# Nicolo2277/Vivim

Measured on AMD Instinct MI355X. Metric: frames/sec fwd+bwd, 256x256 clip=5 3-class, higher is better.
Workload: dtype bf16

## Files before the change

### include/vivim_hip.h

```cpp
#ifndef VIVIM_HIP_H
#define VIVIM_HIP_H

#include <stddef.h>
#include <stdint.h>

#ifdef __cplusplus
extern "C" {
#endif

#define VIVIM_ABI_VERSION 8

typedef enum { VIVIM_F32 = 0, VIVIM_F16 = 1, VIVIM_BF16 = 2 } vivim_dtype_t;

enum {
    VIVIM_OK = 0,
    VIVIM_ERR_INVALID = 1,
    VIVIM_ERR_UNSUPPORTED = 2,
    VIVIM_ERR_LAUNCH = 3
};

typedef struct {
    int32_t batch, dim, seqlen, dstate, n_groups;
    int32_t itype;
    int32_t is_variable_B;
// ... 119 lines not shown
    const void *weight;
    const void *bias;
    void *out;
} vivim_conv_update_params;

typedef struct {
    int32_t batch, dim, dstate;
    int32_t itype;
    int32_t stype;
    int32_t dt_softplus;
    int64_t state_batch_stride, state_d_stride, state_n_stride;
    int64_t x_batch_stride, x_d_stride, dt_batch_stride, dt_d_stride;
    int64_t A_d_stride, A_n_stride;
    int64_t B_batch_stride, B_n_stride, C_batch_stride, C_n_stride;
    int64_t z_batch_stride, z_d_stride, out_batch_stride, out_d_stride;
    void *state;
    const void *x, *dt;
    const void *A;
    const void *B, *C;
    const void *D;
    const void *z;
    const void *dt_bias;
    void *out;
} vivim_state_update_params;

typedef struct {
    int32_t batch, seqlen, channels;
    int32_t itype, otype;
    float eps;
    int64_t x_batch_stride, x_c_stride;
    int64_t y_batch_stride, y_token_stride;
    int64_t dx_batch_stride, dx_c_stride;
    const void *x;
    const void *weight, *bias;
    void *y;
    void *mean, *rstd;
    const void *dy;
    void *dx;
    void *dweight, *dbias;
    void *workspace;
} vivim_layernorm_params;

typedef struct {
    int32_t groups, m, n, k;
    int32_t itype;
    int32_t _pad0;
    int64_t a_group_stride, a_row_stride;
    int64_t b_group_stride, b_row_stride;
    int64_t out_group_stride, out_row_stride;
    const void *a, *b;
    void *out;
} vivim_wgrad_nt_params;

int vivim_abi_version(void);
const char *vivim_last_error(void);

size_t vivim_sizeof(int which);

int vivim_scan_ckpt_len(const vivim_ssm_fwd_params *f);
int vivim_scan_chunk_len(int itype);

size_t vivim_scan_bwd_workspace_bytes(const vivim_ssm_fwd_params *f);
size_t vivim_scan_fwd_workspace_bytes(const vivim_ssm_fwd_params *f);

int vivim_set_tuning(int which, int value);

int vivim_selective_scan_fwd(const vivim_ssm_fwd_params *p, void *stream);
int vivim_selective_scan_bwd(const vivim_ssm_bwd_params *p, void *stream);
int vivim_causal_conv1d_fwd(const vivim_conv_fwd_params *p, void *stream);
int vivim_causal_conv1d_bwd(const vivim_conv_bwd_params *p, void *stream);
int vivim_dwconv_fwd(const vivim_dwconv_params *p, void *stream);
int vivim_dwconv_wgrad(const vivim_dwconv_wgrad_params *p, void *stream);
int vivim_dir_scatter(const vivim_dir_params *p, void *stream);
int vivim_dir_gather(const vivim_dir_params *p, void *stream);
int vivim_causal_conv1d_update(const vivim_conv_update_params *p, void *stream);
int vivim_selective_state_update(const vivim_state_update_params *p, void *stream);
int vivim_layernorm_cm_fwd(const vivim_layernorm_params *p, void *stream);
int vivim_layernorm_cm_bwd(const vivim_layernorm_params *p, void *stream);
size_t vivim_layernorm_bwd_workspace_bytes(const vivim_layernorm_params *p);
int vivim_wgrad_nt(const vivim_wgrad_nt_params *p, void *stream);

size_t vivim_scan_bwd_det_workspace_bytes(const vivim_ssm_fwd_params *f);
size_t vivim_scan_bwd_det_call_workspace_bytes(const vivim_ssm_bwd_params *p);
int vivim_selective_scan_bwd_det(const vivim_ssm_bwd_params *p, void *det_ws, size_t det_ws_bytes, void *stream);

size_t vivim_causal_conv1d_bwd_det_workspace_bytes(const vivim_conv_fwd_params *f);
int vivim_causal_conv1d_bwd_det(const vivim_conv_bwd_params *p, void *det_ws, size_t det_ws_bytes, void *stream);
size_t vivim_dwconv_wgrad_det_workspace_bytes(const vivim_dwconv_wgrad_params *p);
int vivim_dwconv_wgrad_det(const vivim_dwconv_wgrad_params *p, void *det_ws, size_t det_ws_bytes, void *stream);

#ifdef __cplusplus
}
#endif
#endif
```

### vivim_amd/_lib.py

```python
import ctypes
import os
import subprocess

_HERE = os.path.dirname(os.path.abspath(__file__))
CSRC = os.path.join(_HERE, "csrc")
SO_PATH = os.environ.get("VIVIM_LIB") or os.path.join(CSRC, "libvivim_hip.so")

i32, i64, vp = ctypes.c_int32, ctypes.c_int64, ctypes.c_void_p

F32, F16, BF16 = 0, 1, 2


class SsmFwdParams(ctypes.Structure):
    _fields_ = (
        [(n, i32) for n in ("batch", "dim", "seqlen", "dstate", "n_groups", "itype", "is_variable_B",
                            "is_variable_C", "delta_softplus", "_pad0")]
        + [(n, i64) for n in ("u_batch_stride", "u_d_stride", "delta_batch_stride", "delta_d_stride",
                              "z_batch_stride", "z_d_stride", "out_batch_stride", "out_d_stride",
                              "out_z_batch_stride", "out_z_d_stride", "A_d_stride", "A_dstate_stride",
                              "B_batch_stride", "B_group_stride", "B_dstate_stride",
                              "C_batch_stride", "C_group_stride", "C_dstate_stride")]
        + [(n, vp) for n in ("u", "delta", "A", "B", "C", "D", "delta_bias", "z", "out", "out_z", "x", "workspace")]
        + [("workspace_bytes", i64)]
    )
# ... 38 lines not shown
        + [(n, i64) for n in ("x_batch_stride", "x_token_stride", "y_batch_stride", "y_token_stride")]
        + [(n, vp) for n in ("x", "wt", "bias", "y")]
        + [("act", i32), ("_pad1", i32), ("aux", vp), ("aux_batch_stride", i64), ("aux_token_stride", i64)]
    )


class DwConvWgradParams(ctypes.Structure):
    _fields_ = (
        [(n, i32) for n in ("batch", "depth", "height", "width", "channels", "kd", "itype", "_pad0")]
        + [(n, i64) for n in ("x_batch_stride", "x_token_stride", "dy_batch_stride", "dy_token_stride")]
        + [(n, vp) for n in ("x", "dy", "dwt", "dbias")]
    )


class DirParams(ctypes.Structure):
    _fields_ = ([(n, i32) for n in ("batch", "channels", "seqlen", "nframes", "csplit", "itype")]
                + [("scale", ctypes.c_float), ("_pad0", i32)]
                + [(n, i64) for n in ("flat_batch_stride", "flat_c_stride", "stk_batch_stride", "stk_half_stride",
                                      "stk_dir_stride", "stk_c_stride")]
                + [("src", vp), ("dst", vp)])


class ConvUpdateParams(ctypes.Structure):
    _fields_ = ([(n, i32) for n in ("batch", "dim", "width", "itype", "wtype", "silu_activation")]
                + [(n, i64) for n in ("x_batch_stride", "x_c_stride", "state_batch_stride", "state_c_stride",
                                      "state_w_stride", "weight_c_stride", "weight_width_stride",
                                      "out_batch_stride", "out_c_stride")]
                + [(n, vp) for n in ("x", "conv_state", "weight", "bias", "out")])


class StateUpdateParams(ctypes.Structure):
    _fields_ = ([(n, i32) for n in ("batch", "dim", "dstate", "itype", "stype", "dt_softplus")]
                + [(n, i64) for n in ("state_batch_stride", "state_d_stride", "state_n_stride", "x_batch_stride",
                                      "x_d_stride", "dt_batch_stride", "dt_d_stride", "A_d_stride", "A_n_stride",
                                      "B_batch_stride", "B_n_stride", "C_batch_stride", "C_n_stride",
                                      "z_batch_stride", "z_d_stride", "out_batch_stride", "out_d_stride")]
                + [(n, vp) for n in ("state", "x", "dt", "A", "B", "C", "D", "z", "dt_bias", "out")])


class LayerNormParams(ctypes.Structure):
    _fields_ = ([(n, i32) for n in ("batch", "seqlen", "channels", "itype", "otype")] + [("eps", ctypes.c_float)]
                + [(n, i64) for n in ("x_batch_stride", "x_c_stride", "y_batch_stride", "y_token_stride",
                                      "dx_batch_stride", "dx_c_stride")]
                + [(n, vp) for n in ("x", "weight", "bias", "y", "mean", "rstd", "dy", "dx", "dweight", "dbias", "workspace")])


class WgradNtParams(ctypes.Structure):
    _fields_ = ([(n, i32) for n in ("groups", "m", "n", "k", "itype", "_pad0")]
                + [(n, i64) for n in ("a_group_stride", "a_row_stride", "b_group_stride", "b_row_stride",
                                      "out_group_stride", "out_row_stride")]
                + [(n, vp) for n in ("a", "b", "out")])


EXPORTS = ("vivim_abi_version", "vivim_last_error", "vivim_scan_chunk_len", "vivim_scan_ckpt_len", "vivim_sizeof",
           "vivim_scan_bwd_workspace_bytes", "vivim_scan_fwd_workspace_bytes", "vivim_set_tuning",
           "vivim_selective_scan_fwd", "vivim_selective_scan_bwd",
           "vivim_causal_conv1d_fwd", "vivim_causal_conv1d_bwd", "vivim_dwconv_fwd", "vivim_dwconv_wgrad",
           "vivim_dir_scatter", "vivim_dir_gather", "vivim_causal_conv1d_update", "vivim_selective_state_update",
           "vivim_layernorm_cm_fwd", "vivim_layernorm_cm_bwd", "vivim_layernorm_bwd_workspace_bytes", "vivim_wgrad_nt",
           "vivim_scan_bwd_det_workspace_bytes", "vivim_scan_bwd_det_call_workspace_bytes", "vivim_selective_scan_bwd_det",
           "vivim_causal_conv1d_bwd_det_workspace_bytes", "vivim_causal_conv1d_bwd_det",
           "vivim_dwconv_wgrad_det_workspace_bytes", "vivim_dwconv_wgrad_det")

_lib = None


def build(force=False):
    if force:
        subprocess.check_call(["make", "-C", CSRC, "clean"])
    subprocess.check_call(["make", "-C", CSRC, "-j4"])
    return SO_PATH


def lib():
    global _lib
    if _lib is None:
        if not os.path.exists(SO_PATH):
            raise ImportError(
                f"{SO_PATH} is missing: run `python -c 'import __graft_entry__ as g; g.build()'` "
                "(or `make -C vivim_amd/csrc`). vivim_amd has no fallback path.")
        import torch
        L = ctypes.CDLL(SO_PATH)
        L.vivim_last_error.restype = ctypes.c_char_p
        L.vivim_sizeof.restype = ctypes.c_size_t
        L.vivim_sizeof.argtypes = [ctypes.c_int]
        L.vivim_set_tuning.restype = ctypes.c_int
        L.vivim_set_tuning.argtypes = [ctypes.c_int, ctypes.c_int]
        L.vivim_scan_ckpt_len.restype = ctypes.c_int
        L.vivim_scan_ckpt_len.argtypes = [ctypes.POINTER(SsmFwdParams)]
        for fn in (L.vivim_scan_bwd_workspace_bytes, L.vivim_scan_fwd_workspace_bytes):
            fn.restype = ctypes.c_size_t
            fn.argtypes = [ctypes.POINTER(SsmFwdParams)]
        for name, st in (("vivim_selective_scan_fwd", SsmFwdParams), ("vivim_selective_scan_bwd", SsmBwdParams),
                         ("vivim_causal_conv1d_fwd", ConvFwdParams), ("vivim_causal_conv1d_bwd", ConvBwdParams),
                         ("vivim_dwconv_fwd", DwConvParams), ("vivim_dwconv_wgrad", DwConvWgradParams),
                         ("vivim_dir_scatter", DirParams), ("vivim_dir_gather", DirParams),
                         ("vivim_causal_conv1d_update", ConvUpdateParams),
                         ("vivim_selective_state_update", StateUpdateParams),
                         ("vivim_layernorm_cm_fwd", LayerNormParams), ("vivim_layernorm_cm_bwd", LayerNormParams),
                         ("vivim_wgrad_nt", WgradNtParams)):
            fn = getattr(L, name)
            fn.argtypes = [ctypes.POINTER(st), vp]
            fn.restype = ctypes.c_int
        L.vivim_scan_bwd_det_workspace_bytes.restype = ctypes.c_size_t
        L.vivim_scan_bwd_det_workspace_bytes.argtypes = [ctypes.POINTER(SsmFwdParams)]
        for name, st in (("vivim_scan_bwd_det_call_workspace_bytes", SsmBwdParams),
                         ("vivim_causal_conv1d_bwd_det_workspace_bytes", ConvFwdParams),
                         ("vivim_dwconv_wgrad_det_workspace_bytes", DwConvWgradParams)):
            getattr(L, name).restype = ctypes.c_size_t
            getattr(L, name).argtypes = [ctypes.POINTER(st)]
        for name, st in (("vivim_selective_scan_bwd_det", SsmBwdParams), ("vivim_causal_conv1d_bwd_det", ConvBwdParams),
                         ("vivim_dwconv_wgrad_det", DwConvWgradParams)):
            getattr(L, name).argtypes = [ctypes.POINTER(st), vp, ctypes.c_size_t, vp]
            getattr(L, name).restype = ctypes.c_int
        L.vivim_layernorm_bwd_workspace_bytes.argtypes = [ctypes.POINTER(LayerNormParams)]
        L.vivim_layernorm_bwd_workspace_bytes.restype = ctypes.c_size_t
        if L.vivim_abi_version() != 8:
            raise ImportError("libvivim_hip.so ABI version mismatch")
        for which, st in enumerate((SsmFwdParams, SsmBwdParams, ConvFwdParams, ConvBwdParams, DwConvParams,
                                    DwConvWgradParams, DirParams, ConvUpdateParams, StateUpdateParams, LayerNormParams,
                                    WgradNtParams)):
            if L.vivim_sizeof(which) != ctypes.sizeof(st):
                raise ImportError(f"struct layout mismatch for {st.__name__}: "
                                  f"C {L.vivim_sizeof(which)} vs ctypes {ctypes.sizeof(st)}")
        _lib = L
    return _lib


_ISIZE = {F32: 4, F16: 2, BF16: 2}


def algorithmic_bytes(name, P):
    if name.startswith("vivim_selective_scan"):
        f = P.f if name.endswith("bwd") else P
        s = _ISIZE[f.itype]
        act = f.batch * f.dim * f.seqlen * s
        bc = (f.batch * f.n_groups * f.dstate * f.seqlen) if f.is_variable_B else f.dim * f.dstate
        has_z = bool(f.z)
        if name.endswith("fwd"):
            n_act = 3 + (2 if has_z else 0)
            return n_act * act + 2 * bc * (s if f.is_variable_B else 4) + 4 * (f.dim * f.dstate + 2 * f.dim)
        n_act = 5 + (3 if has_z else 0) + (1 if (has_z and f.out_z) else 0)
        return (n_act * act + 2 * bc * (s if f.is_variable_B else 4) + 2 * bc * 4
                + 4 * (2 * f.dim * f.dstate + 4 * f.dim))
    if name.endswith("_update"):
        return 0
    if name.startswith("vivim_dir"):
        return 4 * P.batch * P.channels * P.seqlen * _ISIZE[P.itype]
    if name.startswith("vivim_dwconv"):
        act = P.batch * P.depth * P.height * P.width * P.channels * _ISIZE[P.itype]
        return 2 * act + 4 * P.channels * (P.kd * 9 + 1)
    f = P.f if name.endswith("bwd") else P
    s = _ISIZE[f.itype]
    act = f.batch * f.dim * f.seqlen * s
    if name.endswith("fwd"):
        return 2 * act + 4 * f.dim * (f.width + 1)
    return 3 * act + 8 * f.dim * (f.width + 1)


_profile = None
_event_pool = []
_PROFILED = ("vivim_selective_scan_fwd", "vivim_selective_scan_bwd", "vivim_causal_conv1d_fwd",
             "vivim_causal_conv1d_bwd")


def profile_begin(all_kernels=False):
    global _profile
    _profile = ([], bool(all_kernels))


def profile_end():
    global _profile
    rec = _profile[0] if _profile else []
    _profile = None
# ... 95 lines not shown
```

### vivim_amd/csrc/capi.hip

```cpp
#include <hip/hip_runtime.h>
#include <stdarg.h>
#include <stdio.h>
#include "../../include/vivim_hip.h"
#include "det.cuh"

namespace vivim {
bool conv_fwd_dispatch(const vivim_conv_fwd_params&, hipStream_t);
bool conv_bwd_dispatch(const vivim_conv_bwd_params&, hipStream_t);
bool conv_cl_fwd_dispatch(const vivim_conv_fwd_params&, hipStream_t);
bool conv_cl_bwd_dispatch(const vivim_conv_bwd_params&, hipStream_t);
bool ssm_fwd_dispatch(const vivim_ssm_fwd_params&, hipStream_t);
bool dwconv_fwd_dispatch(const vivim_dwconv_params&, hipStream_t);
bool dwconv_wgrad_dispatch(const vivim_dwconv_wgrad_params&, hipStream_t);
template <bool GATHER> bool dir_dispatch(const vivim_dir_params&, hipStream_t);
void conv_update_launch(const vivim_conv_update_params&, hipStream_t);
void state_update_launch(const vivim_state_update_params&, hipStream_t);
bool ssm_bwd_dispatch(const vivim_ssm_bwd_params&, hipStream_t);
int scan_chunk_len(int itype);
int scan_ckpt_len(const vivim_ssm_fwd_params&);
size_t scan_bwd_workspace_bytes(const vivim_ssm_fwd_params&);
size_t scan_bwd_det_workspace_bytes(const vivim_ssm_fwd_params&);
size_t scan_bwd_det_call_workspace_bytes(const vivim_ssm_bwd_params&);
size_t conv_bwd_det_slots(const vivim_conv_fwd_params&);
bool conv_bwd_det_launch(const vivim_conv_bwd_params&, hipStream_t);
size_t conv_cl_bwd_det_slots(const vivim_conv_fwd_params&);
bool conv_cl_bwd_det_launch(const vivim_conv_bwd_params&, hipStream_t);
size_t dwconv_wgrad_det_workspace_bytes(const vivim_dwconv_wgrad_params&);
int dwconv_wgrad_det_dispatch(const vivim_dwconv_wgrad_params&, void*, size_t, hipStream_t);
int ssm_bwd_det_dispatch(const vivim_ssm_bwd_params&, void* det_ws, size_t det_ws_bytes, hipStream_t);
bool layernorm_dispatch(const vivim_layernorm_params&, bool bwd, hipStream_t);
size_t layernorm_bwd_workspace_bytes(const vivim_layernorm_params&);
bool wgrad_nt_dispatch(const vivim_wgrad_nt_params&, hipStream_t);
size_t scan_fwd_workspace_bytes(const vivim_ssm_fwd_params&);
}

static thread_local char g_err[512] = "";

static int fail(int code, const char* fmt, ...) {
    va_list ap;
    va_start(ap, fmt);
    vsnprintf(g_err, sizeof(g_err), fmt, ap);
    va_end(ap);
    return code;
}

#define VCHECK(cond)                                                                   \
    do {                                                                               \
        if (!(cond)) return fail(VIVIM_ERR_INVALID, "%s: check failed: %s", __func__, #cond); \
    } while (0)

static int after_launch(const char* what) {
    const hipError_t e = hipGetLastError();
    if (e != hipSuccess) return fail(VIVIM_ERR_LAUNCH, "%s: launch failed: %s", what, hipGetErrorString(e));
    return VIVIM_OK;
}

static bool dtype_ok(int t) { return t == VIVIM_F32 || t == VIVIM_F16 || t == VIVIM_BF16; }

static int check_ssm_fwd(const vivim_ssm_fwd_params* p, bool is_bwd) {
    VCHECK(p != nullptr);
    VCHECK(dtype_ok(p->itype));
    VCHECK(p->batch > 0 && p->dim > 0 && p->seqlen > 0 && p->dstate > 0 && p->n_groups > 0);
    VCHECK(p->dstate <= 256);
    VCHECK(p->dim % p->n_groups == 0);
    VCHECK(p->u && p->delta && p->A && p->B && p->C);
    VCHECK(p->x != nullptr || (is_bwd && p->seqlen <= vivim::scan_ckpt_len(*p)));
    if (!is_bwd) VCHECK(p->out != nullptr);
    if (p->z) {
        if (!is_bwd) VCHECK(p->out_z != nullptr);
        else VCHECK(p->out != nullptr);
    }
    if (p->is_variable_B != p->is_variable_C)
        return fail(VIVIM_ERR_UNSUPPORTED,
                    "selective_scan: mixed constant/variable B and C is not built (Vivim uses variable B and C)");
    if (!p->is_variable_B) VCHECK(p->n_groups == 1);
    return VIVIM_OK;
}

namespace vivim {
static int g_tune[2] = {-1, -1};
static int tuning_get(int which, const char* env) {
    int v = __atomic_load_n(&g_tune[which], __ATOMIC_RELAXED);
    if (v < 0) {
        const char* e = getenv(env);
        v = e ? atoi(e) : 0;
        if (v < 0) v = 0;
        __atomic_store_n(&g_tune[which], v, __ATOMIC_RELAXED);
    }
    return v;
}
int tuning_fwd_variant() { return tuning_get(0, "VIVIM_FWD_VARIANT"); }
int tuning_bwd_variant() { return tuning_get(1, "VIVIM_BWD_VARIANT"); }
}

extern "C" {

int vivim_set_tuning(int which, int value) {
    if (which < 0 || which > 1 || value < 0) return -1;
    const int prev = which == 0 ? vivim::tuning_fwd_variant() : vivim::tuning_bwd_variant();
    __atomic_store_n(&vivim::g_tune[which], value, __ATOMIC_RELAXED);
    return prev;
}
int vivim_abi_version(void) { return VIVIM_ABI_VERSION; }
const char* vivim_last_error(void) { return g_err; }
int vivim_scan_chunk_len(int itype) { return vivim::scan_chunk_len(itype); }
int vivim_scan_ckpt_len(const vivim_ssm_fwd_params* f) { return f ? vivim::scan_ckpt_len(*f) : 0; }
size_t vivim_scan_bwd_workspace_bytes(const vivim_ssm_fwd_params* f) {
    return f ? vivim::scan_bwd_workspace_bytes(*f) : 0;
}
size_t vivim_scan_fwd_workspace_bytes(const vivim_ssm_fwd_params* f) {
    return f ? vivim::scan_fwd_workspace_bytes(*f) : 0;
}
size_t vivim_sizeof(int which) {
    switch (which) {
        case 0: return sizeof(vivim_ssm_fwd_params);
        case 1: return sizeof(vivim_ssm_bwd_params);
        case 2: return sizeof(vivim_conv_fwd_params);
        case 3: return sizeof(vivim_conv_bwd_params);
        case 4: return sizeof(vivim_dwconv_params);
        case 5: return sizeof(vivim_dwconv_wgrad_params);
        case 6: return sizeof(vivim_dir_params);
        case 7: return sizeof(vivim_conv_update_params);
        case 8: return sizeof(vivim_state_update_params);
        case 9: return sizeof(vivim_layernorm_params);
        case 10: return sizeof(vivim_wgrad_nt_params);
    }
    return 0;
}

int vivim_selective_scan_fwd(const vivim_ssm_fwd_params* p, void* stream) {
    if (int rc = check_ssm_fwd(p, false)) return rc;
    if (!vivim::ssm_fwd_dispatch(*p, static_cast<hipStream_t>(stream)))
        return fail(VIVIM_ERR_UNSUPPORTED, "selective_scan_fwd not implemented for input type %d", p->itype);
    return after_launch("selective_scan_fwd");
}

static int check_ssm_bwd(const vivim_ssm_bwd_params* p) {
    VCHECK(p != nullptr);
    if (int rc = check_ssm_fwd(&p->f, true)) return rc;
    VCHECK(p->dout && p->du && p->ddelta && p->dA && p->dB && p->dC);
    VCHECK((p->f.D == nullptr) == (p->dD == nullptr));
    VCHECK((p->f.delta_bias == nullptr) == (p->ddelta_bias == nullptr));
    VCHECK((p->f.z == nullptr) == (p->dz == nullptr));
    return VIVIM_OK;
}

int vivim_selective_scan_bwd(const vivim_ssm_bwd_params* p, void* stream) {
    if (int rc = check_ssm_bwd(p)) return rc;
    if (!vivim::ssm_bwd_dispatch(*p, static_cast<hipStream_t>(stream)))
        return fail(VIVIM_ERR_UNSUPPORTED, "selective_scan_bwd not implemented for input type %d", p->f.itype);
    return after_launch("selective_scan_bwd");
}

size_t vivim_scan_bwd_det_workspace_bytes(const vivim_ssm_fwd_params* f) {
    return f && f->batch > 0 && f->dim > 0 && f->seqlen > 0 && f->dstate > 0 && f->n_groups > 0
               ? vivim::scan_bwd_det_workspace_bytes(*f) : 0;
}

size_t vivim_scan_bwd_det_call_workspace_bytes(const vivim_ssm_bwd_params* p) {
    return check_ssm_bwd(p) == VIVIM_OK ? vivim::scan_bwd_det_call_workspace_bytes(*p) : 0;
}

int vivim_selective_scan_bwd_det(const vivim_ssm_bwd_params* p, void* det_ws, size_t det_ws_bytes, void* stream) {
    if (int rc = check_ssm_bwd(p)) return rc;
    switch (vivim::ssm_bwd_det_dispatch(*p, det_ws, det_ws_bytes, static_cast<hipStream_t>(stream))) {
        case 0: break;
        case 2: return fail(VIVIM_ERR_INVALID, "selective_scan_bwd_det: workspace of %zu bytes at %p: need a 16-byte aligned one of "
                            "vivim_scan_bwd_det_call_workspace_bytes() = %zu", det_ws_bytes, det_ws, vivim::scan_bwd_det_call_workspace_bytes(*p));
        default: return fail(VIVIM_ERR_UNSUPPORTED, "selective_scan_bwd_det not implemented for input type %d", p->f.itype);
    }
    return after_launch("selective_scan_bwd_det");
}

static int check_conv(const vivim_conv_fwd_params* p) {
    VCHECK(p != nullptr);
    VCHECK(dtype_ok(p->itype) && dtype_ok(p->wtype));
    VCHECK(p->batch > 0 && p->dim > 0 && p->seqlen > 0);
    VCHECK(p->batch <= 65535 && p->dim <= 65535);
// ... 186 lines not shown
}

static int check_layernorm(const vivim_layernorm_params* p) {
    VCHECK(p != nullptr);
    VCHECK(dtype_ok(p->itype) && (p->otype == VIVIM_F32 || p->otype == p->itype));
    VCHECK(p->batch > 0 && p->seqlen > 0 && p->channels > 0 && p->batch <= 65535);
    if (p->channels > 512)
        return fail(VIVIM_ERR_UNSUPPORTED, "layernorm_cm: more than 512 channels do not fit the backward's two LDS tiles");
    const int64_t e = p->itype == VIVIM_F32 ? 4 : 8;
    VCHECK(p->seqlen % e == 0 && p->x_batch_stride % e == 0 && p->x_c_stride % e == 0);
    VCHECK(p->x && (reinterpret_cast<uintptr_t>(p->x) & 15) == 0 && p->mean && p->rstd);
    return VIVIM_OK;
}

int vivim_layernorm_cm_fwd(const vivim_layernorm_params* p, void* stream) {
    if (int rc = check_layernorm(p)) return rc;
    VCHECK(p->y != nullptr);
    if (!vivim::layernorm_dispatch(*p, false, static_cast<hipStream_t>(stream)))
        return fail(VIVIM_ERR_UNSUPPORTED, "layernorm_cm_fwd not implemented for input type %d / output type %d", p->itype, p->otype);
    return after_launch("layernorm_cm_fwd");
}

size_t vivim_layernorm_bwd_workspace_bytes(const vivim_layernorm_params* p) {
    return p && p->batch > 0 && p->seqlen > 0 && p->channels > 0 ? vivim::layernorm_bwd_workspace_bytes(*p) : 0;
}

int vivim_layernorm_cm_bwd(const vivim_layernorm_params* p, void* stream) {
    if (int rc = check_layernorm(p)) return rc;
    VCHECK(p->dy && p->dx && (reinterpret_cast<uintptr_t>(p->dx) & 15) == 0);
    const int64_t e = p->itype == VIVIM_F32 ? 4 : 8;
    VCHECK(p->dx_batch_stride % e == 0 && p->dx_c_stride % e == 0);
    if ((p->dweight || p->dbias) && !p->workspace)
        return fail(VIVIM_ERR_INVALID, "layernorm_cm_bwd: dweight / dbias need the workspace (vivim_layernorm_bwd_workspace_bytes)");
    if (!vivim::layernorm_dispatch(*p, true, static_cast<hipStream_t>(stream)))
        return fail(VIVIM_ERR_UNSUPPORTED, "layernorm_cm_bwd not implemented for input type %d / output type %d", p->itype, p->otype);
    return after_launch("layernorm_cm_bwd");
}

int vivim_wgrad_nt(const vivim_wgrad_nt_params* p, void* stream) {
    VCHECK(p != nullptr);
    VCHECK(p->groups > 0 && p->groups <= 65535 && p->m > 0 && p->n > 0 && p->k > 0);
    VCHECK(p->a && p->b && p->out);
    if (p->itype != VIVIM_F16 && p->itype != VIVIM_BF16)
        return fail(VIVIM_ERR_UNSUPPORTED, "wgrad_nt takes f16 or bf16 operands (type %d given): f32 products stay on the library GEMM", p->itype);
    VCHECK(p->k % 8 == 0 && p->a_row_stride % 8 == 0 && p->b_row_stride % 8 == 0 && p->a_group_stride % 8 == 0 &&
           p->b_group_stride % 8 == 0);
    VCHECK((reinterpret_cast<uintptr_t>(p->a) & 15) == 0 && (reinterpret_cast<uintptr_t>(p->b) & 15) == 0);
    VCHECK((int64_t)((p->m + 63) / 64) * ((p->n + 15) / 16) <= 65535);
    if (!vivim::wgrad_nt_dispatch(*p, static_cast<hipStream_t>(stream)))
        return fail(VIVIM_ERR_UNSUPPORTED, "wgrad_nt not implemented for type %d", p->itype);
    return after_launch("wgrad_nt");
}

}
```

### vivim_amd/vivim.py

```python
import math

import os

import torch
import torch.nn as nn
import torch.nn.functional as F

from . import dwconv as _dw
from . import layernorm as _ln
from .mamba_simple import Mamba


class DropPath(nn.Module):

    def __init__(self, drop_prob=0.0):
        super().__init__()
        self.drop_prob = drop_prob

    def forward(self, x):
        if self.drop_prob == 0.0 or not self.training:
            return x
        keep = 1.0 - self.drop_prob
        mask = x.new_empty((x.shape[0],) + (1,) * (x.dim() - 1)).bernoulli_(keep).div_(keep)
        return x * mask


def _init_weights(m):
    if isinstance(m, nn.Linear):
        nn.init.trunc_normal_(m.weight, std=0.02)
        if m.bias is not None:
            nn.init.constant_(m.bias, 0)
    elif isinstance(m, nn.LayerNorm):
        nn.init.constant_(m.bias, 0)
        nn.init.constant_(m.weight, 1.0)
    elif isinstance(m, nn.Conv2d):
        fan_out = m.kernel_size[0] * m.kernel_size[1] * m.out_channels // m.groups
        m.weight.data.normal_(0, math.sqrt(2.0 / fan_out))
        if m.bias is not None:
            m.bias.data.zero_()


class LayerNorm(nn.Module):

    def __init__(self, normalized_shape, eps=1e-6, data_format="channels_last"):
        super().__init__()
        if data_format not in ("channels_last", "channels_first"):
            raise NotImplementedError
        self.weight = nn.Parameter(torch.ones(normalized_shape))
        self.bias = nn.Parameter(torch.zeros(normalized_shape))
        self.eps = eps
        self.data_format = data_format
        self.normalized_shape = (normalized_shape,)

    def forward(self, x):
        if self.data_format == "channels_last":
            return F.layer_norm(x, self.normalized_shape, self.weight, self.bias, self.eps)
        mean = x.mean(1, keepdim=True)
        var = (x - mean).pow(2).mean(1, keepdim=True)
        x = (x - mean) / torch.sqrt(var + self.eps)
        return self.weight[:, None, None] * x + self.bias[:, None, None]


class DWConv(nn.Module):

    def __init__(self, dim=768):
        super().__init__()
        self.dwconv = nn.Conv3d(dim, dim, 3, 1, 1, bias=True, groups=dim)

    def forward(self, x, nf, H, W):
        B, _, C = x.shape
        if _dw.supported(x, self.dwconv.weight):
            return _dw.depthwise_conv_tokens(x, self.dwconv.weight, self.dwconv.bias, nf, H, W)
        x = self.dwconv(x.transpose(1, 2).view(B, C, nf, H, W))
        return x.flatten(2).transpose(1, 2)


class Mlp(nn.Module):
    def __init__(self, in_features, hidden_features=None, out_features=None, act_layer=nn.GELU, drop=0.0):
        super().__init__()
        out_features = out_features or in_features
        hidden_features = hidden_features or in_features
        self.fc1 = nn.Linear(in_features, hidden_features)
        self.dwconv = DWConv(hidden_features)
        self.act = act_layer()
        self.fc2 = nn.Linear(hidden_features, out_features)
        self.drop = nn.Dropout(drop)
        self.apply(_init_weights)

    def forward(self, x, nf, H, W):
        x = self.fc1(x)
        conv = self.dwconv.dwconv
        if isinstance(self.act, nn.GELU) and self.act.approximate == "none" and _dw.supported(x, conv.weight) \
                and not os.environ.get("VIVIM_NO_DWCONV_GELU"):
            x = self.drop(_dw.depthwise_conv_gelu_tokens(x, conv.weight, conv.bias, nf, H, W))
        else:
            x = self.drop(self.act(self.dwconv(x, nf, H, W)))
        return self.drop(self.fc2(x))


class MambaLayer(nn.Module):

    def __init__(self, dim, d_state=16, d_conv=4, expand=2, mlp_ratio=4, drop=0.0, drop_path=0.0,
                 act_layer=nn.GELU):
        super().__init__()
        self.dim = dim
        self.norm1 = nn.LayerNorm(dim)
        self.mamba = Mamba(d_model=dim, d_state=d_state, d_conv=d_conv, expand=expand, bimamba_type="v3")
        self.drop_path = DropPath(drop_path) if drop_path > 0.0 else nn.Identity()
        self.norm2 = nn.LayerNorm(dim)
        self.mlp = Mlp(in_features=dim, hidden_features=int(dim * mlp_ratio), act_layer=act_layer, drop=drop)
        self.apply(_init_weights)

    @staticmethod
    def _norm(norm, x_flat):
        if (_ln.supported(x_flat, norm.weight) and _ln.worthwhile(x_flat)
                and not os.environ.get("VIVIM_NO_FUSED_LAYERNORM")):
            return _ln.layer_norm_cm(x_flat, norm.weight, norm.bias, norm.eps)
        return norm(x_flat)

    def forward(self, x):
        B, C, nf, H, W = x.shape
        assert C == self.dim
        x_flat = x.reshape(B, C, nf * H * W).transpose(-1, -2)
        x_flat = x_flat + self.drop_path(self.mamba(self._norm(self.norm1, x_flat), nframes=nf))
        x_flat = x_flat + self.drop_path(self.mlp(self._norm(self.norm2, x_flat), nf, H, W))
        return x_flat.transpose(-1, -2).reshape(B, C, nf, H, W)


def _encoder_parts(backbone):
    seg = backbone.segformer
    if hasattr(seg, "encoder"):
        enc = seg.encoder
        return list(enc.patch_embeddings), list(enc.block), list(enc.layer_norm)
    return ([s.patch_embeddings for s in seg.stages], [s.blocks for s in seg.stages],
            [s.layer_norm for s in seg.stages])


class _TokenDWConv2d(nn.Module):
# ... 7 lines not shown
            return _dw.depthwise_conv_tokens(hidden_states, self.dwconv.weight, self.dwconv.bias, 1, height, width)
        b, _, c = hidden_states.shape
        y = self.dwconv(hidden_states.transpose(1, 2).view(b, c, height, width))
        return y.flatten(2).transpose(1, 2)


def _swap_backbone_dwconv(module):
    n = 0
    for m in module.modules():
        inner = getattr(m, "dwconv", None)
        conv = getattr(inner, "dwconv", None)
        if isinstance(conv, nn.Conv2d) and conv.groups == conv.in_channels and conv.kernel_size == (3, 3) \
                and conv.stride == (1, 1) and conv.padding == (1, 1) and not isinstance(inner, _TokenDWConv2d):
            m.dwconv = _TokenDWConv2d(inner)
            n += 1
    return n


def _swap_backbone_droppath(module):
    n = 0
    for m in module.modules():
        dp = getattr(m, "drop_path", None)
        if isinstance(dp, nn.Module) and type(dp).__name__ == "SegformerDropPath":
            m.drop_path = DropPath(float(dp.drop_prob))
            n += 1
    return n


class _Encoder(nn.Module):

    def __init__(self, backbone):
        super().__init__()
        pe, blocks, norms = _encoder_parts(backbone)
        self.patch_embeddings = nn.ModuleList(pe)
        self.block = nn.ModuleList(blocks)
        self.layer_norm = nn.ModuleList(norms)


def _run_block(blk, hs, height, width):
    out = blk(hs, height, width)
    return out[0] if isinstance(out, (tuple, list)) else out


class mamba_block(nn.Module):

    def __init__(self, backbone, in_chans=1, depths=[2, 2, 2, 2], dims=[64, 128, 320, 512],
                 drop_path_rate=0.0, layer_scale_init_value=1e-6, out_indices=[0, 1, 2, 3], mamba_kwargs=None,
                 fast_backbone_dwconv=False):
        super().__init__()
        self.downsample_layers = _Encoder(backbone)
        if fast_backbone_dwconv:
            _swap_backbone_dwconv(self.downsample_layers)
            _swap_backbone_droppath(self.downsample_layers)
        dp_rates = [x.item() for x in torch.linspace(0, drop_path_rate, sum(depths))]
        mk = mamba_kwargs or {}
        self.stages = nn.ModuleList()
        for i in range(len(dims)):
            self.stages.append(nn.Sequential(*[nn.Sequential(MambaLayer(dim=dims[i], drop_path=dp_rates[i], **mk))
                                               for _ in range(depths[i])]))
        self.out_indices = out_indices

    def forward_features(self, x):
        bz, nf = x.shape[:2]
        hs = x.reshape(bz * nf, *x.shape[-3:])
        outs = []
        enc = self.downsample_layers
        for embed, blocks, _norm, mam_stage in zip(enc.patch_embeddings, enc.block, enc.layer_norm, self.stages):
            hs, height, width = embed(hs)
            for blk in blocks:
                hs = _run_block(blk, hs, height, width)
            hs = hs.reshape(bz * nf, height, width, -1).permute(0, 3, 1, 2).contiguous()
            hs = hs.reshape(bz, nf, *hs.shape[-3:]).transpose(1, 2)
            hs = mam_stage(hs)
            hs = hs.transpose(1, 2).reshape(bz * nf, hs.shape[1], height, width)
            outs.append(hs)
        return tuple(outs)

    def forward(self, x):
        return self.forward_features(x)


def segformer_b3_config(num_labels=150):
    from transformers import SegformerConfig
    return SegformerConfig(num_channels=3, num_encoder_blocks=4, depths=[3, 4, 18, 3], sr_ratios=[8, 4, 2, 1],
                           hidden_sizes=[64, 128, 320, 512], patch_sizes=[7, 3, 3, 3], strides=[4, 2, 2, 2],
                           num_attention_heads=[1, 2, 5, 8], mlp_ratios=[4, 4, 4, 4], decoder_hidden_size=768,
                           num_labels=num_labels)


def segformer_b3_random(num_labels=150):
    from transformers import SegformerForSemanticSegmentation
    return SegformerForSemanticSegmentation(segformer_b3_config(num_labels))


class Vivim(nn.Module):

    def __init__(self, in_chans=3, out_chans=3, depths=[2, 2, 2, 2], feat_size=[64, 128, 320, 512],
                 drop_path_rate=0.2, layer_scale_init_value=1e-6, hidden_size: int = 768, norm_name="instance",
                 conv_block: bool = True, res_block: bool = True, spatial_dims=2, with_edge=False,
                 dropout_rate=0.3, backbone=None, mamba_kwargs=None, fast_backbone_dwconv=False) -> None:
        super().__init__()
        self.hidden_size = hidden_size
        self.in_chans, self.out_chans = in_chans, out_chans
        self.depths, self.feat_size = depths, feat_size
        self.drop_path_rate = drop_path_rate
        self.layer_scale_init_value = layer_scale_init_value
        self.dropout_rate = dropout_rate
        self.spatial_dims = spatial_dims
        if backbone is None:
            from transformers import SegformerForSemanticSegmentation
            backbone = SegformerForSemanticSegmentation.from_pretrained("nvidia/segformer-b3-finetuned-ade-512-512")
        self.encoder = mamba_block(backbone, in_chans, depths=depths, dims=feat_size,
                                   drop_path_rate=drop_path_rate, mamba_kwargs=mamba_kwargs,
                                   fast_backbone_dwconv=fast_backbone_dwconv)
        self.decoder = backbone.decode_head
        self.feature_dropout = nn.Dropout2d(dropout_rate)
        self.out = nn.Conv2d(768, out_chans, kernel_size=1)
        self.with_edge = with_edge
        if with_edge:
            self.edgeocr_cls_head = nn.Conv2d(64, 1, kernel_size=1, stride=1, padding=0, bias=True)

    def _decoder_projections(self):
        dec = self.decoder
        return dec.linear_c if hasattr(dec, "linear_c") else dec.linear_projections

    def decode(self, encoder_hidden_states, bz, nf):
        batch_size = encoder_hidden_states[-1].shape[0]
        size0 = encoder_hidden_states[0].shape[2:]
        feats = ()
        for state, mlp in zip(encoder_hidden_states, self._decoder_projections()):
            height, width = state.shape[2], state.shape[3]
            state = mlp(state).permute(0, 2, 1).reshape(batch_size, -1, height, width)
            state = F.interpolate(state, size=size0, mode="bilinear", align_corners=False)
            if torch.rand(1).item() > 0.5:
                state = F.dropout(state, p=self.dropout_rate / 2, training=self.training)
            feats += (state,)
        hidden = self.decoder.linear_fuse(torch.cat(feats[::-1], dim=1))
        hidden = self.decoder.activation(self.decoder.batch_norm(hidden))
        hidden = self.decoder.dropout(self.decoder.dropout(hidden))
        hidden = self.feature_dropout(hidden)
        return self.out(hidden)

    def forward(self, x_in):
        bz, nf, nc, h, w = x_in.shape
        outs = self.encoder(x_in)
        logits = F.interpolate(self.decode(outs, bz, nf), size=(h, w), mode="bilinear", align_corners=False)
        if self.with_edge:
            edge = F.interpolate(self.edgeocr_cls_head(outs[0]), size=(h, w), mode="bilinear", align_corners=False)
            return logits, edge
        return logits
```

Before: 216.6.

## Add MFMA split-K linear weight-gradient kernel with fused bias reduction

New measurement: 210.9. 2.6% lower.

```diff
diff --git a/include/vivim_hip.h b/include/vivim_hip.h
--- a/include/vivim_hip.h
+++ b/include/vivim_hip.h
@@ -195,6 +195,19 @@
     void *out;
 } vivim_wgrad_nt_params;
 
+typedef struct {
+    int32_t tokens, cout, cin;
+    int32_t itype;
+    int32_t tokens_per_clip;
+    int32_t min_steps;
+    int64_t dy_row_stride, dy_token_stride, dy_clip_stride;
+    int64_t x_row_stride, x_token_stride, x_clip_stride;
+    int64_t dw_row_stride;
+    const void *dy, *x;
+    void *dw;
+    void *db;
+} vivim_linear_wgrad_params;
+
 int vivim_abi_version(void);
 const char *vivim_last_error(void);
 
@@ -222,6 +235,7 @@
 int vivim_layernorm_cm_bwd(const vivim_layernorm_params *p, void *stream);
 size_t vivim_layernorm_bwd_workspace_bytes(const vivim_layernorm_params *p);
 int vivim_wgrad_nt(const vivim_wgrad_nt_params *p, void *stream);
+int vivim_linear_wgrad(const vivim_linear_wgrad_params *p, void *stream);
 
 size_t vivim_scan_bwd_det_workspace_bytes(const vivim_ssm_fwd_params *f);
 size_t vivim_scan_bwd_det_call_workspace_bytes(const vivim_ssm_bwd_params *p);
diff --git a/vivim_amd/_lib.py b/vivim_amd/_lib.py
--- a/vivim_amd/_lib.py
+++ b/vivim_amd/_lib.py
@@ -114,12 +114,20 @@
                 + [(n, vp) for n in ("a", "b", "out")])
 
 
+class LinearWgradParams(ctypes.Structure):
+    _fields_ = ([(n, i32) for n in ("tokens", "cout", "cin", "itype", "tokens_per_clip", "min_steps")]
+                + [(n, i64) for n in ("dy_row_stride", "dy_token_stride", "dy_clip_stride",
+                                      "x_row_stride", "x_token_stride", "x_clip_stride", "dw_row_stride")]
+                + [(n, vp) for n in ("dy", "x", "dw", "db")])
+
+
 EXPORTS = ("vivim_abi_version", "vivim_last_error", "vivim_scan_chunk_len", "vivim_scan_ckpt_len", "vivim_sizeof",
            "vivim_scan_bwd_workspace_bytes", "vivim_scan_fwd_workspace_bytes", "vivim_set_tuning",
            "vivim_selective_scan_fwd", "vivim_selective_scan_bwd",
            "vivim_causal_conv1d_fwd", "vivim_causal_conv1d_bwd", "vivim_dwconv_fwd", "vivim_dwconv_wgrad",
            "vivim_dir_scatter", "vivim_dir_gather", "vivim_causal_conv1d_update", "vivim_selective_state_update",
            "vivim_layernorm_cm_fwd", "vivim_layernorm_cm_bwd", "vivim_layernorm_bwd_workspace_bytes", "vivim_wgrad_nt",
+           "vivim_linear_wgrad",
            "vivim_scan_bwd_det_workspace_bytes", "vivim_scan_bwd_det_call_workspace_bytes", "vivim_selective_scan_bwd_det",
            "vivim_causal_conv1d_bwd_det_workspace_bytes", "vivim_causal_conv1d_bwd_det",
            "vivim_dwconv_wgrad_det_workspace_bytes", "vivim_dwconv_wgrad_det")
@@ -160,7 +168,7 @@
                          ("vivim_causal_conv1d_update", ConvUpdateParams),
                          ("vivim_selective_state_update", StateUpdateParams),
                          ("vivim_layernorm_cm_fwd", LayerNormParams), ("vivim_layernorm_cm_bwd", LayerNormParams),
-                         ("vivim_wgrad_nt", WgradNtParams)):
+                         ("vivim_wgrad_nt", WgradNtParams), ("vivim_linear_wgrad", LinearWgradParams)):
             fn = getattr(L, name)
             fn.argtypes = [ctypes.POINTER(st), vp]
             fn.restype = ctypes.c_int
@@ -181,7 +189,7 @@
             raise ImportError("libvivim_hip.so ABI version mismatch")
         for which, st in enumerate((SsmFwdParams, SsmBwdParams, ConvFwdParams, ConvBwdParams, DwConvParams,
                                     DwConvWgradParams, DirParams, ConvUpdateParams, StateUpdateParams, LayerNormParams,
-                                    WgradNtParams)):
+                                    WgradNtParams, LinearWgradParams)):
             if L.vivim_sizeof(which) != ctypes.sizeof(st):
                 raise ImportError(f"struct layout mismatch for {st.__name__}: "
                                   f"C {L.vivim_sizeof(which)} vs ctypes {ctypes.sizeof(st)}")
diff --git a/vivim_amd/csrc/capi.hip b/vivim_amd/csrc/capi.hip
--- a/vivim_amd/csrc/capi.hip
+++ b/vivim_amd/csrc/capi.hip
@@ -31,6 +31,7 @@
 bool layernorm_dispatch(const vivim_layernorm_params&, bool bwd, hipStream_t);
 size_t layernorm_bwd_workspace_bytes(const vivim_layernorm_params&);
 bool wgrad_nt_dispatch(const vivim_wgrad_nt_params&, hipStream_t);
+bool linear_wgrad_dispatch(const vivim_linear_wgrad_params&, hipStream_t);
 size_t scan_fwd_workspace_bytes(const vivim_ssm_fwd_params&);
 }
 
@@ -124,6 +125,7 @@
         case 8: return sizeof(vivim_state_update_params);
         case 9: return sizeof(vivim_layernorm_params);
         case 10: return sizeof(vivim_wgrad_nt_params);
+        case 11: return sizeof(vivim_linear_wgrad_params);
     }
     return 0;
 }
@@ -416,4 +418,24 @@
     return after_launch("wgrad_nt");
 }
 
-}
+int vivim_linear_wgrad(const vivim_linear_wgrad_params* p, void* stream) {
+    VCHECK(p != nullptr);
+    VCHECK(p->tokens > 0 && p->cout > 0 && p->cin > 0 && p->min_steps >= 0);
+    VCHECK(p->tokens_per_clip > 0 && p->tokens % p->tokens_per_clip == 0);
+    VCHECK(p->dy && p->x && p->dw);
+    if (p->itype != VIVIM_F16 && p->itype != VIVIM_BF16)
+        return fail(VIVIM_ERR_UNSUPPORTED, "linear_wgrad takes f16 or bf16 operands (type %d given): f32 products stay on the library GEMM", p->itype);
+    if (p->dy_row_stride != 1 || p->x_row_stride != 1)
+        return fail(VIVIM_ERR_UNSUPPORTED, "linear_wgrad: only token-major operands (channel stride 1) are built");
+    VCHECK(p->cout % 8 == 0 && p->cin % 8 == 0);
+    VCHECK(p->dy_token_stride % 8 == 0 && p->dy_clip_stride % 8 == 0 && p->x_token_stride % 8 == 0 && p->x_clip_stride % 8 == 0);
+    VCHECK(p->dy_token_stride >= p->cout && p->x_token_stride >= p->cin && p->dw_row_stride >= p->cin);
+    VCHECK((reinterpret_cast<uintptr_t>(p->dy) & 15) == 0 && (reinterpret_cast<uintptr_t>(p->x) & 15) == 0);
+    VCHECK((reinterpret_cast<uintptr_t>(p->dw) & 3) == 0 && (reinterpret_cast<uintptr_t>(p->db) & 3) == 0);
+    VCHECK((int64_t)((p->cout + 63) / 64) * ((p->cin + 63) / 64) <= 65535);
+    if (!vivim::linear_wgrad_dispatch(*p, static_cast<hipStream_t>(stream)))
+        return fail(VIVIM_ERR_UNSUPPORTED, "linear_wgrad not implemented for type %d", p->itype);
+    return after_launch("linear_wgrad");
+}
+
+}
diff --git a/vivim_amd/csrc/linear_wgrad.hip b/vivim_amd/csrc/linear_wgrad.hip
--- /dev/null
+++ b/vivim_amd/csrc/linear_wgrad.hip
@@ -0,0 +1,164 @@
+#include "common.cuh"
+
+namespace vivim {
+
+typedef __attribute__((ext_vector_type(8))) __bf16 lw_bf8;
+typedef __attribute__((ext_vector_type(8))) _Float16 lw_h8;
+typedef __attribute__((ext_vector_type(4))) float lw_f4;
+typedef __attribute__((ext_vector_type(4))) short lw_s4;
+typedef __attribute__((ext_vector_type(8))) short lw_s8;
+typedef __attribute__((ext_vector_type(4))) unsigned lw_u4;
+
+template <typename T> struct LwFrag;
+template <> struct LwFrag<bf16_t> {
+    typedef lw_bf8 type;
+    static constexpr short kOne = 0x3F80;
+    static __device__ __forceinline__ lw_f4 mma(type a, type b, lw_f4 c) { return __builtin_amdgcn_mfma_f32_16x16x32_bf16(a, b, c, 0, 0, 0); }
+};
+template <> struct LwFrag<f16_t> {
+    typedef lw_h8 type;
+    static constexpr short kOne = 0x3C00;
+    static __device__ __forceinline__ lw_f4 mma(type a, type b, lw_f4 c) { return __builtin_amdgcn_mfma_f32_16x16x32_f16(a, b, c, 0, 0, 0); }
+};
+
+constexpr int kLwFrags = 4;
+constexpr int kLwTile = 16 * kLwFrags;
+constexpr int kLwStep = 32;
+constexpr int kLwRow = 160;
+constexpr int kLwImage = kLwStep * kLwRow;
+constexpr int kLwLoads = 4;
+constexpr int kLwDepth = 3;
+
+typedef __attribute__((address_space(3))) lw_s4* lw_lds_s4;
+
+template <typename T>
+__global__ void __launch_bounds__(kWave) linear_wgrad_kernel(const vivim_linear_wgrad_params p, const int steps_per_split, const int col_tiles) {
+    typedef typename LwFrag<T>::type frag;
+    __shared__ __attribute__((aligned(16))) unsigned char lds[2 * kLwImage];
+    const int lane = threadIdx.x;
+    const int rt = blockIdx.y / col_tiles, ct = blockIdx.y - rt * col_tiles;
+    const int m0 = rt * kLwTile, n0 = ct * kLwTile;
+    const bool bias = p.db != nullptr && ct == 0;
+
+    const int lrow = lane >> 3, lch = 8 * (lane & 7);
+    const bool a_in = m0 + lch < p.cout, b_in = n0 + lch < p.cin;
+    const T* __restrict__ a = static_cast<const T*>(p.dy) + m0 + (a_in ? lch : 0);
+    const T* __restrict__ b = static_cast<const T*>(p.x) + n0 + (b_in ? lch : 0);
+    const unsigned tpc = (unsigned)p.tokens_per_clip;
+    const int nsteps = (p.tokens + kLwStep - 1) / kLwStep;
+    const int s0 = blockIdx.x * steps_per_split, s1 = min(nsteps, s0 + steps_per_split);
+    auto load = [&](lw_u4 (&ra)[kLwLoads], lw_u4 (&rb)[kLwLoads], int s) -> unsigned {
+        unsigned inside = 0;
+#pragma unroll
+        for (int n = 0; n < kLwLoads; ++n) {
+            const unsigned t = (unsigned)(kLwStep * s + lrow + 8 * n);
+            inside |= (s < s1 && t < (unsigned)p.tokens ? 1u : 0u) << n;
+            const unsigned tc = min(t, (unsigned)p.tokens - 1u);
+            const unsigned clip = tc / tpc, tok = tc - clip * tpc;
+            ra[n] = *reinterpret_cast<const lw_u4*>(a + (int64_t)clip * p.dy_clip_stride + (int64_t)tok * p.dy_token_stride);
+            rb[n] = *reinterpret_cast<const lw_u4*>(b + (int64_t)clip * p.x_clip_stride + (int64_t)tok * p.x_token_stride);
+        }
+        return inside;
+    };
+    const int wr_off = lrow * kLwRow + 2 * lch;
+    const int kq = lane >> 4, q = (lane >> 2) & 3, pp = lane & 3;
+    const int rd_off = (16 * (kq >> 1) + 4 * (kq & 1) + q) * kLwRow + 8 * pp;
+    auto fragment = [&](int image, int f) -> frag {
+        const lw_s4 lo = __builtin_amdgcn_ds_read_tr16_b64_v4i16((lw_lds_s4)(lds + image + rd_off + 32 * f));
+        const lw_s4 hi = __builtin_amdgcn_ds_read_tr16_b64_v4i16((lw_lds_s4)(lds + image + rd_off + 32 * f + 8 * kLwRow));
+        return __builtin_bit_cast(frag, __builtin_shufflevector(lo, hi, 0, 1, 2, 3, 4, 5, 6, 7));
+    };
+
+    lw_f4 acc[kLwFrags][kLwFrags], accb[kLwFrags];
+#pragma unroll
+    for (int i = 0; i < kLwFrags; ++i) {
+        accb[i] = lw_f4{0.f, 0.f, 0.f, 0.f};
+#pragma unroll
+        for (int j = 0; j < kLwFrags; ++j) acc[i][j] = lw_f4{0.f, 0.f, 0.f, 0.f};
+    }
+    constexpr short kOne = LwFrag<T>::kOne;
+    const frag ones = __builtin_bit_cast(frag, lw_s8{kOne, kOne, kOne, kOne, kOne, kOne, kOne, kOne});
+
+    const lw_u4 zero = {0u, 0u, 0u, 0u};
+    lw_u4 ra[kLwDepth][kLwLoads], rb[kLwDepth][kLwLoads];
+    unsigned inside[kLwDepth];
+#pragma unroll
+    for (int d = 0; d < kLwDepth - 1; ++d) inside[d] = load(ra[d], rb[d], s0 + d);
+    for (int s = s0; s < s1; s += kLwDepth) {
+#pragma unroll
+        for (int h = 0; h < kLwDepth; ++h) {
+            const int nxt = (h + kLwDepth - 1) % kLwDepth;
+            inside[nxt] = load(ra[nxt], rb[nxt], s + h + kLwDepth - 1);
+#pragma unroll
+            for (int n = 0; n < kLwLoads; ++n) {
+                const bool in = (inside[h] >> n) & 1u;
+                *reinterpret_cast<lw_u4*>(lds + wr_off + 8 * n * kLwRow) = in && a_in ? ra[h][n] : zero;
+                *reinterpret_cast<lw_u4*>(lds + kLwImage + wr_off + 8 * n * kLwRow) = in && b_in ? rb[h][n] : zero;
+            }
+            __builtin_amdgcn_fence(__ATOMIC_RELEASE, "wavefront");
+            __builtin_amdgcn_wave_barrier();
+            __builtin_amdgcn_fence(__ATOMIC_ACQUIRE, "wavefront");
+            frag fa[kLwFrags], fb[kLwFrags];
+#pragma unroll
+            for (int i = 0; i < kLwFrags; ++i) fa[i] = fragment(0, i);
+#pragma unroll
+            for (int j = 0; j < kLwFrags; ++j) fb[j] = fragment(kLwImage, j);
+            __builtin_amdgcn_fence(__ATOMIC_RELEASE, "wavefront");
+            __builtin_amdgcn_wave_barrier();
+            __builtin_amdgcn_fence(__ATOMIC_ACQUIRE, "wavefront");
+#pragma unroll
+            for (int i = 0; i < kLwFrags; ++i)
+#pragma unroll
+                for (int j = 0; j < kLwFrags; ++j) acc[i][j] = LwFrag<T>::mma(fa[i], fb[j], acc[i][j]);
+            if (bias) {
+#pragma unroll
+                for (int i = 0; i < kLwFrags; ++i) accb[i] = LwFrag<T>::mma(fa[i], ones, accb[i]);
+            }
+        }
+    }
+    float* __restrict__ dw = static_cast<float*>(p.dw);
+    const int r = lane & 15;
+#pragma unroll
+    for (int i = 0; i < kLwFrags; ++i) {
+#pragma unroll
+        for (int e = 0; e < 4; ++e) {
+            const int row = m0 + 16 * i + 4 * kq + e;
+            if (row < p.cout) {
+#pragma unroll
+                for (int j = 0; j < kLwFrags; ++j) {
+                    const int col = n0 + 16 * j + r;
+                    if (col < p.cin) atomicAdd(dw + (int64_t)row * p.dw_row_stride + col, acc[i][j][e]);
+                }
+                if (bias && r == 0) atomicAdd(static_cast<float*>(p.db) + row, accb[i][e]);
+            }
+        }
+    }
+}
+
+static int lw_splits(const vivim_linear_wgrad_params& p, int* steps_per_split) {
+    const int row_tiles = (p.cout + kLwTile - 1) / kLwTile, col_tiles = (p.cin + kLwTile - 1) / kLwTile;
+    const int nsteps = (p.tokens + kLwStep - 1) / kLwStep;
+    const int minsteps = p.min_steps > 0 ? p.min_steps : 16;
+    int splits = std::min(std::max(1, 2048 / (row_tiles * col_tiles)), std::max(1, nsteps / minsteps));
+    const int sps = (nsteps + splits - 1) / splits;
+    *steps_per_split = sps;
+    return (nsteps + sps - 1) / sps;
+}
+
+template <typename T>
+static void lw_launch(const vivim_linear_wgrad_params& p, hipStream_t stream) {
+    const int row_tiles = (p.cout + kLwTile - 1) / kLwTile, col_tiles = (p.cin + kLwTile - 1) / kLwTile;
+    int sps;
+    const int splits = lw_splits(p, &sps);
+    hipLaunchKernelGGL((linear_wgrad_kernel<T>), dim3(splits, row_tiles * col_tiles), dim3(kWave), 0, stream, p, sps, col_tiles);
+}
+
+bool linear_wgrad_dispatch(const vivim_linear_wgrad_params& p, hipStream_t stream) {
+    switch (p.itype) {
+        case VIVIM_BF16: lw_launch<bf16_t>(p, stream); return true;
+        case VIVIM_F16: lw_launch<f16_t>(p, stream); return true;
+    }
+    return false;
+}
+
+}
diff --git a/vivim_amd/linear.py b/vivim_amd/linear.py
--- /dev/null
+++ b/vivim_amd/linear.py
@@ -0,0 +1,126 @@
+import os
+
+import torch
+import torch.nn as nn
+import torch.nn.functional as F
+
+from . import _lib
+
+_ITYPE = {torch.float16: _lib.F16, torch.bfloat16: _lib.BF16}
+MIN_TOKENS = 8192
+
+
+def _compute_dtype(x, weight):
+    if torch.is_autocast_enabled("cuda"):
+        dt = torch.get_autocast_dtype("cuda")
+        return dt if dt in _ITYPE and x.is_floating_point() else None
+    return x.dtype if x.dtype in _ITYPE and weight.dtype == x.dtype else None
+
+
+def _tokens(t):
+    if t.dim() < 2 or t.stride(-1) != 1 or t.data_ptr() % 16:
+        return None
+    if t.dim() > 3:
+        if not t.is_contiguous():
+            return None
+        t = t.view(-1, t.shape[-1])
+    if t.dim() == 2:
+        T, tpc, ts, cs = t.shape[0], t.shape[0], t.stride(0), 0
+    elif t.stride(0) == t.shape[1] * t.stride(1) or t.shape[0] == 1:
+        T, tpc, ts, cs = t.shape[0] * t.shape[1], t.shape[0] * t.shape[1], t.stride(1), 0
+    else:
+        T, tpc, ts, cs = t.shape[0] * t.shape[1], t.shape[1], t.stride(1), t.stride(0)
+    if T == 0 or ts % 8 or cs % 8 or ts < t.shape[-1] or T >= 2 ** 31:
+        return None
+    return T, tpc, ts, cs
+
+
+def supported(x, weight, bias=None):
+    if x.numel() < MIN_TOKENS * x.shape[-1]:
+        return False
+    if os.environ.get("VIVIM_NO_LINEAR_WGRAD") or _lib.deterministic():
+        return False
+    if not (x.is_cuda and weight.is_cuda and torch.is_grad_enabled() and weight.requires_grad and weight.dim() == 2):
+        return False
+    if _compute_dtype(x, weight) is None or weight.dtype not in (torch.float32, torch.float16, torch.bfloat16):
+        return False
+    if bias is not None and bias.dtype != weight.dtype:
+        return False
+    cout, cin = weight.shape
+    if cout % 8 or cin % 8 or x.shape[-1] != cin:
+        return False
+    tk = _tokens(x)
+    return tk is not None and tk[0] >= MIN_TOKENS
+
+
+def linear_wgrad(dy, x, with_bias, min_steps=0):
+    tdy, tx = _tokens(dy), _tokens(x)
+    if tdy is None or tx is None or tdy[0] != tx[0] or dy.dtype not in _ITYPE or x.dtype != dy.dtype:
+        return None
+    T, tpc = tx[0], min(tdy[1], tx[1])
+    if (tdy[1] != T and tdy[1] != tpc) or (tx[1] != T and tx[1] != tpc):
+        return None
+    cout, cin = dy.shape[-1], x.shape[-1]
+    buf = _lib.zeros(cout * (cin + 1), x.device)
+    P = _lib.LinearWgradParams()
+    P.tokens, P.cout, P.cin, P.itype, P.tokens_per_clip, P.min_steps = T, cout, cin, _ITYPE[x.dtype], tpc, min_steps
+    P.dy_row_stride, P.dy_token_stride, P.dy_clip_stride = 1, tdy[2], (tdy[3] if tdy[1] == tpc and tpc != T else tpc * tdy[2])
+    P.x_row_stride, P.x_token_stride, P.x_clip_stride = 1, tx[2], (tx[3] if tx[1] == tpc and tpc != T else tpc * tx[2])
+    P.dw_row_stride = cin
+    P.dy, P.x, P.dw = dy.data_ptr(), x.data_ptr(), buf.data_ptr()
+    P.db = P.dw + 4 * cout * cin if with_bias else None
+    if x.device.index == torch.cuda.current_device():
+        _lib.call("vivim_linear_wgrad", P, torch.cuda.current_stream().cuda_stream)
+    else:
+        with torch.cuda.device(x.device):
+            _lib.call("vivim_linear_wgrad", P, torch.cuda.current_stream().cuda_stream)
+    return buf[:cout * cin].view(cout, cin), (buf[cout * cin:] if with_bias else None)
+
+
+class _Linear(torch.autograd.Function):
+    @staticmethod
+    @torch.amp.custom_fwd(device_type="cuda")
+    def forward(ctx, x, weight, bias, dtype):
+        x16, w16 = x.to(dtype), weight.to(dtype)
+        b16 = bias.to(dtype) if bias is not None else None
+        ctx.save_for_backward(x16, w16)
+        ctx.x_dtype, ctx.w_dtype, ctx.has_bias = x.dtype, weight.dtype, bias is not None
+        return F.linear(x16, w16, b16)
+
+    @staticmethod
+    @torch.amp.custom_bwd(device_type="cuda")
+    def backward(ctx, dy):
+        x16, w16 = ctx.saved_tensors
+        dx = dy.matmul(w16).to(ctx.x_dtype) if ctx.needs_input_grad[0] else None
+        got = linear_wgrad(dy, x16, ctx.has_bias)
+        if got is None:
+            dy2 = dy.reshape(-1, dy.shape[-1])
+            dw = dy2.t().matmul(x16.reshape(-1, x16.shape[-1]))
+            db = dy2.sum(0) if ctx.has_bias else None
+        else:
+            dw, db = got
+        if dw.dtype != ctx.w_dtype:
+            dw = dw.to(ctx.w_dtype)
+            db = db.to(ctx.w_dtype) if db is not None else None
+        return dx, dw, db, None
+
+
+def linear(x, weight, bias=None):
+    return _Linear.apply(x, weight, bias, _compute_dtype(x, weight))
+
+
+class Linear(nn.Linear):
+
+    def forward(self, x):
+        if supported(x, self.weight, self.bias):
+            return linear(x, self.weight, self.bias)
+        return F.linear(x, self.weight, self.bias)
+
+
+def swap_linears(module):
+    n = 0
+    for m in module.modules():
+        if type(m) is nn.Linear:
+            m.__class__ = Linear
+            n += 1
+    return n
diff --git a/vivim_amd/vivim.py b/vivim_amd/vivim.py
--- a/vivim_amd/vivim.py
+++ b/vivim_amd/vivim.py
@@ -8,6 +8,7 @@
 
 from . import dwconv as _dw
 from . import layernorm as _ln
+from . import linear as _lin
 from .mamba_simple import Mamba
 
 
@@ -80,10 +81,10 @@
         super().__init__()
         out_features = out_features or in_features
         hidden_features = hidden_features or in_features
-        self.fc1 = nn.Linear(in_features, hidden_features)
+        self.fc1 = _lin.Linear(in_features, hidden_features)
         self.dwconv = DWConv(hidden_features)
         self.act = act_layer()
-        self.fc2 = nn.Linear(hidden_features, out_features)
+        self.fc2 = _lin.Linear(hidden_features, out_features)
         self.drop = nn.Dropout(drop)
         self.apply(_init_weights)
 
@@ -197,6 +198,7 @@
         if fast_backbone_dwconv:
             _swap_backbone_dwconv(self.downsample_layers)
             _swap_backbone_droppath(self.downsample_layers)
+            _lin.swap_linears(self.downsample_layers)
         dp_rates = [x.item() for x in torch.linspace(0, drop_path_rate, sum(depths))]
         mk = mamba_kwargs or {}
         self.stages = nn.ModuleList()
@@ -259,6 +261,8 @@
                                    drop_path_rate=drop_path_rate, mamba_kwargs=mamba_kwargs,
                                    fast_backbone_dwconv=fast_backbone_dwconv)
         self.decoder = backbone.decode_head
+        if fast_backbone_dwconv:
+            _lin.swap_linears(self.decoder)
         self.feature_dropout = nn.Dropout2d(dropout_rate)
         self.out = nn.Conv2d(768, out_chans, kernel_size=1)
         self.with_edge = with_edge
```
